# ZooMEISTER/vickers-hardness-Unet

Measured on AMD Instinct MI355X. Metric: 512x512 images/sec (train fwd+bwd), higher is better.
Workload: dtype bf16

## Files before the change

### include/vk_unet.h

```cpp
#ifndef VK_UNET_H
#define VK_UNET_H

#include <stddef.h>
#include <stdint.h>

#ifdef __cplusplus
extern "C" {
#endif

#define VK_ABI_VERSION 1
#define VK_STATS_REPLICAS 32

typedef enum { VK_F32 = 0, VK_BF16 = 1, VK_F16 = 2 } vk_dtype;

enum { VK_OK = 0, VK_ERR_ARG = -1, VK_ERR_STATE = -2, VK_ERR_UNSUPPORTED = -3 };

int vk_version(void);
const char* vk_last_error_string(void);
int vk_has_gfx950_code(void);
int vk_probe_mfma_rate(int iters, int waves_per_simd, float* sink, double* flops_out, void* stream);
int vk_set_reserved_cus(int n);
int vk_debug_hold_cus(int workgroups, int threads, int lds_bytes, int microseconds, const void* traffic, size_t traffic_bytes,
                      float* sink, void* stream);

// ... 377 lines not shown
                               const float* found_inf, float* scratch, void* stream);
#define VK_ADAMW_MAX_GROUPS 8
typedef struct {
  float lr, beta1, beta2, eps, weight_decay;
} vk_adamw_group;
int vk_adamw_step_groups(int n_segments, const int64_t* segments, const int32_t* segment_group, int n_blocks, const int32_t* blocks,
                         float* param, const float* grad, float* exp_avg, float* exp_avg_sq, int n_groups,
                         const vk_adamw_group* groups_host, int* step_counts, float inv_scale, const float* grad_scale,
                         const float* found_inf, const float* clip_coef, float* scratch, void* stream);
#define VK_NORM_L2 0
#define VK_NORM_INF 1
int vk_grad_norm_segments(int n_segments, const int64_t* segments, int n_blocks, const int32_t* blocks, const float* grad,
                          int norm_kind, float inv_scale, float max_norm, double* partials, float* out, void* stream);

typedef struct vk_unet vk_unet;

typedef struct {
  int N, size;
  vk_dtype dtype;
  int training;
  int width;
} vk_unet_config;

typedef struct {
  char name[96];
  int kind;
  int dims[4];
  int ndim;
  int64_t offset;
  int64_t numel;
} vk_tensor_info;

int vk_unet_create(const vk_unet_config* cfg, vk_unet** out);
int vk_unet_create_ex(const vk_unet_config* cfg, int classes, vk_unet** out);
int vk_unet_num_classes(const vk_unet* h);
#define VK_ENC_RESNET18 18
#define VK_ENC_RESNET34 34
#define VK_ENC_RESNET50 50
int vk_unet_create_enc(const vk_unet_config* cfg, int classes, int encoder, vk_unet** out);
int vk_unet_encoder(const vk_unet* h);
void vk_unet_destroy(vk_unet* h);
int vk_unet_set_side_stream(vk_unet* h, int enable);
int vk_unet_num_tensors(const vk_unet* h);
int vk_unet_tensor_info(const vk_unet* h, int index, vk_tensor_info* out);
int64_t vk_unet_param_numel(const vk_unet* h);
int64_t vk_unet_buffer_numel(const vk_unet* h);
int64_t vk_unet_workspace_bytes(const vk_unet* h);
int vk_unet_num_buckets(const vk_unet* h);
int vk_unet_bucket_range(const vk_unet* h, int bucket, int64_t* elem_begin, int64_t* elem_end);

int vk_unet_bind(vk_unet* h, float* params, float* grads, float* bn_buffers, int64_t* nbt, void* workspace,
                 size_t workspace_bytes);
int vk_unet_refresh_weights(vk_unet* h, void* stream);

int vk_unet_forward(vk_unet* h, const float* x, float* logits, int training, void* stream);
int vk_unet_loss(vk_unet* h, const float* logits, const float* target, float* loss_out, float grad_scale,
                 float w_bce, float w_dice, void* stream);
#define VK_LOSS_BINARY 0
#define VK_LOSS_MULTILABEL 1
#define VK_LOSS_MULTICLASS 2
int vk_unet_loss_ex(vk_unet* h, int mode, const void* logits, const void* target, float* loss_out, float grad_scale, float w_ce,
                    float w_dice, void* stream);
int vk_unet_loss_cfg(vk_unet* h, const vk_seg_loss_cfg* cfg, const void* logits, const void* target, float* loss_out,
                     float grad_scale, void* stream);
int vk_unet_loss_lovasz(vk_unet* h, const vk_seg_loss_cfg* seg_cfg, const vk_lovasz_cfg* lovasz_cfg, float w_lovasz, const void* logits,
                        const void* target, void* workspace, size_t workspace_bytes, float* loss_out, float grad_scale, void* stream);
int vk_unet_backward(vk_unet* h, const float* dlogits, int stage_begin, int stage_end, void* stream);
int vk_unet_set_trainable(vk_unet* h, const uint8_t* flags, int n);
int vk_unet_set_bn_frozen(vk_unet* h, const uint8_t* flags, int n);
int vk_unet_set_input_grad(vk_unet* h, float* dx);
int vk_unet_zero_grad(vk_unet* h, void* stream);

#define VK_COMM_ID_BYTES 128
typedef struct vk_comm vk_comm;
int vk_comm_unique_id(void* id_out );
int vk_comm_init(int rank, int world, const void* id, vk_comm** out);
int vk_comm_world(const vk_comm* c);
int vk_allreduce_bucket(vk_comm* c, float* grads, size_t count, void* stream);
int vk_comm_broadcast(vk_comm* c, void* buf, size_t bytes, int root, void* stream);
int vk_comm_destroy(vk_comm* c);

int vk_unet_debug_tensor(const vk_unet* h, const char* name, void** ptr, int dims_nhwc[4]);

#ifdef __cplusplus
}
#endif
#endif
```

### vickers-hardness-unet_amd/_lib.py

```python
from __future__ import annotations

import ctypes as C
import os
import subprocess
from pathlib import Path

PKG_DIR = Path(__file__).resolve().parent
LIB_PATH = Path(os.environ["VK_LIB"]) if os.environ.get("VK_LIB") else PKG_DIR / "libvkunet.so"
CSRC = PKG_DIR / "csrc"

VK_F32, VK_BF16, VK_F16 = 0, 1, 2
VK_LOSS_BINARY, VK_LOSS_MULTILABEL, VK_LOSS_MULTICLASS = 0, 1, 2
VK_ENC_RESNET18, VK_ENC_RESNET34, VK_ENC_RESNET50 = 18, 34, 50
VK_ADAMW_MAX_GROUPS = 8
VK_NORM_L2, VK_NORM_INF = 0, 1
VK_TILE_MAX_ORIGINS, VK_TILE_MAX_SIDE = 64, 4096
VK_BLEND_PROB, VK_BLEND_LOGIT = 0, 1
VK_PATCH_FORCE_GENERAL = 1


class VkError(RuntimeError):
    pass


# ... 4 lines not shown

class vk_conv_desc(C.Structure):
    _fields_ = [("dtype", C.c_int), ("N", C.c_int), ("H", C.c_int), ("W", C.c_int), ("Ho", C.c_int),
                ("Wo", C.c_int), ("K", C.c_int), ("R", C.c_int), ("S", C.c_int), ("stride", C.c_int),
                ("pad", C.c_int), ("transposed", C.c_int), ("src0", vk_src), ("src1", vk_src)]


class vk_bnr(C.Structure):
    _fields_ = [("z", C.c_void_p), ("scale", C.c_void_p), ("shift", C.c_void_p), ("sums", C.c_void_p), ("mask", C.c_void_p),
                ("accumulate", C.c_int)]


class vk_letterbox_desc(C.Structure):
    _fields_ = [("h", C.c_int), ("w", C.c_int), ("src_stride", C.c_int), ("size", C.c_int), ("nh", C.c_int),
                ("nw", C.c_int), ("top", C.c_int), ("left", C.c_int), ("pad_value", C.c_int)]


class vk_tile_desc(C.Structure):
    _fields_ = [("h", C.c_int), ("w", C.c_int), ("src_stride", C.c_int), ("T", C.c_int), ("overlap", C.c_int), ("ny", C.c_int),
                ("nx", C.c_int), ("ys", C.c_int * VK_TILE_MAX_ORIGINS), ("xs", C.c_int * VK_TILE_MAX_ORIGINS), ("view_mask", C.c_int),
                ("pad_value", C.c_int), ("C", C.c_int)]


class vk_geom_desc(C.Structure):
    _fields_ = [("h", C.c_int), ("w", C.c_int), ("bin_thresh", C.c_float), ("morph_kernel", C.c_int), ("open_iter", C.c_int),
                ("close_iter", C.c_int), ("min_area", C.c_int), ("max_components", C.c_int)]


class vk_geom_det(C.Structure):
    _fields_ = [("label", C.c_int), ("area", C.c_int), ("box", C.c_int * 8), ("cx", C.c_float), ("cy", C.c_float),
                ("rw", C.c_float), ("rh", C.c_float), ("ux", C.c_float), ("uy", C.c_float), ("hull_n", C.c_int),
                ("reserved", C.c_int), ("d1", C.c_double), ("d2", C.c_double), ("d_mean", C.c_double)]


class vk_geom_quad(C.Structure):
    _fields_ = [("label", C.c_int), ("area", C.c_int), ("box", C.c_int * 8), ("cx", C.c_float), ("cy", C.c_float),
                ("valid", C.c_int), ("branch", C.c_int), ("n_candidates", C.c_int), ("contour_n", C.c_int), ("hull_n", C.c_int),
                ("flags", C.c_int), ("quality", C.c_double), ("d1", C.c_double), ("d2", C.c_double), ("d_mean", C.c_double)]


class vk_aug_params(C.Structure):
    _fields_ = [("d4", C.c_int), ("rotate", C.c_int), ("cos_a", C.c_float), ("sin_a", C.c_float), ("photo", C.c_int),
                ("alpha", C.c_float), ("beta", C.c_float), ("blur_ksize", C.c_int), ("noise_scale", C.c_float),
                ("noise_seed", C.c_uint32), ("clahe_limit", C.c_int)]


class vk_patch_item(C.Structure):
    _fields_ = [("img_off", C.c_int64), ("msk_off", C.c_int64), ("h", C.c_int), ("w", C.c_int), ("row_off", C.c_int64)]


class vk_patch_params(C.Structure):
    _fields_ = [("item", C.c_int), ("k", C.c_int), ("oy", C.c_int), ("ox", C.c_int), ("zoom", C.c_float), ("cos_a", C.c_float),
                ("sin_a", C.c_float), ("reserved", C.c_int)]


class vk_seg_loss_cfg(C.Structure):
    _fields_ = [("struct_size", C.c_uint32), ("mode", C.c_int32), ("terms", C.c_uint32), ("has_ignore", C.c_int32),
                ("ignore_index", C.c_int32), ("w_pix", C.c_float), ("w_focal", C.c_float), ("w_dice", C.c_float),
                ("w_jaccard", C.c_float), ("w_tversky", C.c_float), ("pix_smooth", C.c_float), ("pix_denom_valid", C.c_int32),
                ("has_pos_weight", C.c_int32), ("pos_weight", C.c_float * 16), ("focal_has_alpha", C.c_int32),
                ("focal_alpha", C.c_float), ("focal_gamma", C.c_float),
                ("dice_smooth", C.c_float), ("dice_eps", C.c_float), ("dice_log", C.c_int32), ("dice_classes", C.c_uint32),
                ("jaccard_smooth", C.c_float), ("jaccard_eps", C.c_float), ("jaccard_log", C.c_int32), ("jaccard_classes", C.c_uint32),
                ("tversky_smooth", C.c_float), ("tversky_eps", C.c_float), ("tversky_log", C.c_int32), ("tversky_classes", C.c_uint32),
                ("tversky_alpha", C.c_float), ("tversky_beta", C.c_float), ("tversky_gamma", C.c_float),
                ("w_mcc", C.c_float), ("mcc_eps", C.c_float)]


class vk_lovasz_cfg(C.Structure):
    _fields_ = [("struct_size", C.c_uint32), ("mode", C.c_int32), ("per_image", C.c_int32), ("has_ignore", C.c_int32),
                ("ignore_index", C.c_int32)]


SWEEP_FIELDS = ("stats", "per_image", "dice", "iou", "mean_dice", "mean_iou", "micro_stats", "micro", "ap", "auc", "best_dice", "best_iou",
                "best_f1", "best_mean", "group_dice", "group_iou", "group_mean_dice", "group_mean_iou", "epoch_dice", "epoch_iou",
                "epoch_mean_dice", "epoch_mean_iou")


class vk_sweep_layout(C.Structure):
    _fields_ = [(f, C.c_size_t) for f in SWEEP_FIELDS + ("total_bytes", "workspace_bytes")]


INST_INT_FIELDS = ("tp", "fp", "fn", "n_rel", "n_pred_used", "n_gt_used", "n_split", "n_merge", "overflow_pred", "overflow_gt", "n_images")
INST_FLOAT_FIELDS = ("sum_iou", "sum_abs_d", "sum_rel_d", "sum_signed_rel_d", "sum_hv_rel", "max_abs_d")


class vk_inst_stats(C.Structure):
    _fields_ = [(f, C.c_int64) for f in INST_INT_FIELDS] + [(f, C.c_double) for f in INST_FLOAT_FIELDS]


VK_SUBPIX_CORNER, VK_SUBPIX_LINES = 0, 1
VK_SUBPIX_MAX_WIN, VK_SUBPIX_MAX_REACH, VK_SUBPIX_MAX_STATIONS = 15, 15, 32
SUBPIX_FLAGS = {"singular": 1, "left_map": 2, "not_converged": 4, "restored": 8, "short_side": 16, "no_edge": 32, "parallel": 64}


class vk_subpix_params(C.Structure):
    _fields_ = [("method", C.c_int), ("win", C.c_int), ("zero_zone", C.c_int), ("max_iter", C.c_int), ("eps", C.c_double),
                ("wt", C.c_double * (2 * VK_SUBPIX_MAX_WIN + 1)), ("n_stations", C.c_int), ("reach", C.c_int), ("lo", C.c_double),
                ("hi", C.c_double), ("level", C.c_double), ("max_shift", C.c_double)]


class vk_subpix_quad(C.Structure):
    _fields_ = [("label", C.c_int), ("area", C.c_int), ("valid", C.c_int), ("reserved", C.c_int), ("flags", C.c_int * 4),
                ("iters", C.c_int * 4), ("v", C.c_double * 8), ("vs", C.c_double * 8), ("d1", C.c_double), ("d2", C.c_double),
                ("d_mean", C.c_double)]

# ... 75 lines not shown
    "vk_head_fwd": (ci, [ci, ci, ci, ci, P(vk_src), vp, vp, vp, vp]),
    "vk_dec4_tail_eval": (ci, [ci, ci, ci, ci, P(vk_src), vp, vp, vp, vp, vp, vp, vp, vp, vp, vp]),
    "vk_head_bwd": (ci, [ci, ci, ci, ci, P(vk_src), vp, vp, vp, vp, vp, vp, sz, vp]),
    "vk_bce_dice_loss": (ci, [sz, vp, vp, vp, vp, vp, cf, cf, cf, vp]),
    "vk_head_fwd_multi": (ci, [ci, ci, ci, ci, ci, P(vk_src), vp, vp, vp, vp]),
    "vk_head_multi_workspace_bytes": (sz, [ci]),
    "vk_head_bwd_multi": (ci, [ci, ci, ci, ci, ci, P(vk_src), vp, vp, vp, vp, vp, P(vk_bnr), vp, sz, vp]),
    "vk_multi_loss_workspace_bytes": (sz, [ci, ci, ci]),
    "vk_multilabel_loss": (ci, [ci, ci, ci, vp, vp, vp, sz, vp, vp, cf, cf, cf, vp]),
    "vk_multiclass_loss": (ci, [ci, ci, ci, vp, vp, vp, sz, vp, vp, cf, cf, cf, vp]),
    "vk_seg_loss_cfg_size": (sz, []),
    "vk_seg_loss_workspace_bytes": (sz, [ci, ci, ci]),
    "vk_seg_loss": (ci, [P(vk_seg_loss_cfg), ci, ci, ci, vp, vp, vp, sz, vp, vp, cf, vp]),
    "vk_lovasz_cfg_size": (sz, []),
    "vk_lovasz_workspace_bytes": (sz, [P(vk_lovasz_cfg), ci, ci, ci]),
    "vk_lovasz_loss": (ci, [P(vk_lovasz_cfg), ci, ci, ci, vp, vp, vp, sz, vp, vp, cf, ci, vp]),
    "vk_lovasz_flat_workspace_bytes": (sz, [ci, i64]),
    "vk_lovasz_flat": (ci, [vp, vp, ci, i64, vp, sz, vp, vp, vp, vp]),
    "vk_seg_metrics_workspace_bytes": (C.c_size_t, [ci]),
    "vk_seg_metrics": (ci, [ci, sz, vp, vp, ci, cf, cf, vp, sz, vp, vp]),
    "vk_seg_metrics_multi_workspace_bytes": (sz, [ci, ci]),
    "vk_seg_metrics_multi": (ci, [ci, ci, ci, sz, vp, vp, ci, cf, cf, vp, sz, vp, vp, vp, vp]),
    "vk_sweep_hist": (ci, [ci, sz, sz, vp, vp, ci, ci, ci, ci, ci, vp, vp, ci, vp, vp, vp]),
    "vk_sweep_curves_layout": (ci, [ci, ci, ci, ci, P(vk_sweep_layout)]),
    "vk_sweep_curves_out_bytes": (sz, [ci, ci, ci, ci]),
    "vk_sweep_curves": (ci, [ci, ci, ci, vp, vp, ci, cf, vp, sz, vp, sz, vp]),
    "vk_inst_contingency": (ci, [ci, ci, ci, vp, vp, ci, ci, vp, vp]),
    "vk_inst_match": (ci, [ci, ci, ci, vp, vp, vp, ci, vp, vp, sz, vp, sz, vp, vp, vp, vp, vp, ci, vp]),
    "vk_subpix_refine": (ci, [P(vk_subpix_params), ci, ci, ci, vp, vp, sz, sz, ci, vp, ci, vp, vp, vp]),
    "vk_adamw_step": (ci, [sz, vp, vp, vp, vp, cf, cf, cf, cf, cf, ci, cf, vp, vp, ci, vp]),
    "vk_amp_check_inf": (ci, [sz, vp, vp, vp]),
    "vk_amp_unscale_check": (ci, [sz, vp, vp, vp, vp]),
    "vk_adamw_step_amp": (ci, [sz, vp, vp, vp, vp, cf, cf, cf, cf, cf, vp, cf, vp, vp, vp, vp, ci, vp]),
    "vk_adamw_segment_blocks": (ci, [ci, P(i64), P(C.c_int32), ci]),
    "vk_adamw_step_amp_segments": (ci, [ci, vp, ci, vp, vp, vp, vp, vp, cf, cf, cf, cf, cf, vp, cf, vp, vp, vp, vp]),
    "vk_adamw_step_groups": (ci, [ci, vp, vp, ci, vp, vp, vp, vp, vp, ci, P(vk_adamw_group), vp, cf, vp, vp, vp, vp, vp]),
    "vk_grad_norm_segments": (ci, [ci, vp, ci, vp, vp, ci, cf, cf, vp, vp, vp]),
    "vk_unet_create": (ci, [P(vk_unet_config), P(vp)]),
    "vk_unet_create_ex": (ci, [P(vk_unet_config), ci, P(vp)]),
    "vk_unet_num_classes": (ci, [vp]),
    "vk_unet_create_enc": (ci, [P(vk_unet_config), ci, ci, P(vp)]),
    "vk_unet_encoder": (ci, [vp]),
    "vk_unet_destroy": (None, [vp]),
    "vk_unet_set_side_stream": (ci, [vp, ci]),
    "vk_unet_num_tensors": (ci, [vp]),
    "vk_unet_tensor_info": (ci, [vp, ci, P(vk_tensor_info)]),
    "vk_unet_param_numel": (i64, [vp]),
    "vk_unet_buffer_numel": (i64, [vp]),
    "vk_unet_workspace_bytes": (i64, [vp]),
    "vk_unet_num_buckets": (ci, [vp]),
    "vk_unet_bucket_range": (ci, [vp, ci, P(i64), P(i64)]),
    "vk_unet_bind": (ci, [vp, vp, vp, vp, vp, vp, sz]),
    "vk_unet_refresh_weights": (ci, [vp, vp]),
    "vk_unet_forward": (ci, [vp, vp, vp, ci, vp]),
    "vk_unet_loss": (ci, [vp, vp, vp, vp, cf, cf, cf, vp]),
    "vk_unet_loss_ex": (ci, [vp, ci, vp, vp, vp, cf, cf, cf, vp]),
    "vk_unet_loss_cfg": (ci, [vp, P(vk_seg_loss_cfg), vp, vp, vp, cf, vp]),
    "vk_unet_loss_lovasz": (ci, [vp, P(vk_seg_loss_cfg), P(vk_lovasz_cfg), cf, vp, vp, vp, sz, vp, cf, vp]),
    "vk_unet_backward": (ci, [vp, vp, ci, ci, vp]),
    "vk_unet_set_trainable": (ci, [vp, P(C.c_uint8), ci]),
    "vk_unet_set_bn_frozen": (ci, [vp, P(C.c_uint8), ci]),
    "vk_unet_set_input_grad": (ci, [vp, vp]),
    "vk_unet_zero_grad": (ci, [vp, vp]),
    "vk_unet_debug_tensor": (ci, [vp, C.c_char_p, P(vp), P(ci * 4)]),
    "vk_comm_unique_id": (ci, [vp]),
    "vk_comm_init": (ci, [ci, ci, vp, P(vp)]),
    "vk_comm_world": (ci, [vp]),
    "vk_allreduce_bucket": (ci, [vp, vp, sz, vp]),
    "vk_comm_broadcast": (ci, [vp, vp, sz, ci, vp]),
    "vk_comm_destroy": (ci, [vp]),
}

_lib = None


def build(force: bool = False, verbose: bool = False) -> Path:
    srcs = list(CSRC.glob("*.hip")) + list(CSRC.glob("*.h")) + [PKG_DIR.parent / "include" / "vk_unet.h"]
    if not force and LIB_PATH.exists() and all(LIB_PATH.stat().st_mtime >= s.stat().st_mtime for s in srcs):
        return LIB_PATH
    hipcc = os.environ.get("HIPCC", "/opt/rocm/bin/hipcc")
    if not Path(hipcc).exists():
        raise VkError(f"hipcc not found at {hipcc}; cannot build libvkunet.so")
    cmd = ["make", "-C", str(CSRC), f"-j{min(4, os.cpu_count() or 1)}", f"HIPCC={hipcc}"]
    r = subprocess.run(cmd, capture_output=True, text=True)
    if verbose:
        print(r.stdout[-2000:], r.stderr[-2000:])
    if r.returncode != 0 or not LIB_PATH.exists():
        raise VkError("building libvkunet.so failed:\n" + r.stdout[-3000:] + r.stderr[-3000:])
    return LIB_PATH


def lib():
    global _lib
    if _lib is not None:
        return _lib
    if not LIB_PATH.exists():
        raise VkError(f"{LIB_PATH} is missing: build it with __graft_entry__.build() "
                      f"(make -C {CSRC}); this package has no CPU fallback")
    try:
        L = C.CDLL(str(LIB_PATH))
    except OSError as e:
        raise VkError(f"cannot load {LIB_PATH}: {e}") from e
    for name, (res, args) in SIGNATURES.items():
        fn = getattr(L, name, None)
        if fn is None:
            raise VkError(f"{LIB_PATH} does not export {name}")
# ... 38 lines not shown
```

### vickers-hardness-unet_amd/csrc/engine.hip

```cpp
#include <stdarg.h>
#include <stdio.h>
#include <stdlib.h>
#include <string.h>

#include <algorithm>
#include <atomic>
#include <map>
#include <mutex>
#include <string>
#include <vector>

#include "vk_common.h"

namespace vkh {
static thread_local char g_err[512] = "";
void set_error(const char* fmt, ...) {
  va_list ap;
  va_start(ap, fmt);
  vsnprintf(g_err, sizeof(g_err), fmt, ap);
  va_end(ap);
}

struct ProfRec {
  std::string tag;
// ... 183 lines not shown
    if (!e.transposed) {
      pos = (int)(v & 3);
      long t = v >> 2;
      k = (int)(t % rows); t /= rows;
      tap = (int)(t % 9); cc = (int)(t / 9);
    } else {
      k = (int)(v % rows);
      long t = v / rows;
      pos = (int)(t & 3); t >>= 2;
      tap = (int)(t % 9); cc = (int)(t / 9);
    }
    const int j = pos ^ (((k >> 2) & 1) << 1);
    const int r0 = cc * CK + j * VE;
    float f[VE];
    if (!e.transposed) {
      const f32x4_t* s4 = reinterpret_cast<const f32x4_t*>(src + ((long)k * 9 + tap) * red + r0);
#pragma unroll
      for (int q = 0; q < VE / 4; ++q) {
        const f32x4_t t = s4[q];
#pragma unroll
        for (int i = 0; i < 4; ++i) f[4 * q + i] = t[i];
      }
    } else {
#pragma unroll
      for (int i = 0; i < VE; ++i) f[i] = src[((long)(r0 + i) * 9 + tap) * rows + k];
    }
    dst[(((long)cc * 9 + tap) * rows + k) * 4 + pos] = Vec16<T>::pack(f);
  }
}

template <typename T>
__global__ void k_cast_flat(size_t n, const float* __restrict__ src, T* __restrict__ dst) {
  for (size_t i = blockIdx.x * (size_t)blockDim.x + threadIdx.x; i < n; i += (size_t)gridDim.x * blockDim.x) st1(dst + i, src[i]);
}

struct CastRange {
  int64_t begin, count;
};
template <typename T>
__global__ void k_cast_ranges(const CastRange* __restrict__ tab, const float* __restrict__ src, T* __restrict__ dst) {
  const CastRange r = tab[blockIdx.y];
  for (int64_t i = blockIdx.x * (int64_t)blockDim.x + threadIdx.x; i < r.count; i += (int64_t)gridDim.x * blockDim.x)
    st1(dst + r.begin + i, src[r.begin + i]);
}

template <typename T>
__global__ void k_pack_stem(const float* __restrict__ w, T* __restrict__ wp) {
  const int i = blockIdx.x * blockDim.x + threadIdx.x;
  if (i >= 64 * 7 * 32) return;
  const int j = i % 32, r = (i / 32) % 7, k = i / (32 * 7);
  const int s = j >> 2, c = j & 3;
  const float v = (s < 7 && c < 3) ? w[((k * 7 + r) * 7 + s) * 3 + c] : 0.f;
  st1(wp + i, v);
}

struct BnEvalEntry {
  int64_t g_off, b_off, rm_off, rv_off, out_off;
  int C, pad_;
};
__global__ void k_bn_eval_all(const BnEvalEntry* __restrict__ tab, const float* __restrict__ params, const float* __restrict__ bufs,
                              float* __restrict__ arena, float eps) {
  const BnEvalEntry e = tab[blockIdx.x];
  for (int c = threadIdx.x; c < e.C; c += blockDim.x) {
    const float invstd = (float)(1.0 / sqrt((double)bufs[e.rv_off + c] + (double)eps));
    const float sc = params[e.g_off + c] * invstd;
    arena[e.out_off + c] = sc;
    arena[e.out_off + e.C + c] = params[e.b_off + c] - bufs[e.rm_off + c] * sc;
  }
}

__global__ void k_inc_i64(int n, int64_t* p) {
  const int i = blockIdx.x * blockDim.x + threadIdx.x;
  if (i < n) p[i] += 1;
}

__global__ void k_inc_i64_masked(int n, int64_t* p, uint64_t frozen) {
  const int i = blockIdx.x * blockDim.x + threadIdx.x;
  if (i < n && !((frozen >> i) & 1ull)) p[i] += 1;
}

__global__ void k_bn_frozen_affine(const BnEvalEntry* __restrict__ tab, uint64_t frozen, const float* __restrict__ params,
                                   const float* __restrict__ bufs, float* __restrict__ arena, float eps) {
  if (!((frozen >> blockIdx.x) & 1ull)) return;
  const BnEvalEntry e = tab[blockIdx.x];
  float* f = arena + e.out_off;
  for (int c = threadIdx.x; c < e.C; c += blockDim.x) {
    const float invstd = (float)(1.0 / sqrt((double)bufs[e.rv_off + c] + (double)eps));
    const float sc = params[e.g_off + c] * invstd;
    f[c] = sc;
    f[e.C + c] = params[e.b_off + c] - bufs[e.rm_off + c] * sc;
    f[2 * e.C + c] = bufs[e.rm_off + c];
    f[3 * e.C + c] = invstd;
    f[4 * e.C + c] = sc;
    f[5 * e.C + c] = 0.f;
    f[6 * e.C + c] = 0.f;
  }
}

struct ConvL {
  std::string name;
  int Cin, K, R, stride, pad;
  int64_t w_off;
  int64_t wd_off;
  bool halo_fwd = false;
  bool halo_dg = false;
  int bn;
// ... 81 lines not shown
  int sink_c = 512;
  int eb;
  std::vector<vk_tensor_info> infos;
  int n_ptensors = 0;
  std::vector<uint8_t> trainable;
  int last_rank = 0;
  uint64_t bn_frozen = 0, bn_frozen_fwd = 0;
  float* dx_in = nullptr;
  int input_rank = 0;
  unsigned mask_version = 0;
  std::vector<ConvL> convs;
  std::vector<BnL> bns;
  std::vector<BlockL> blocks;
  std::vector<DecL> decs;
  int stem_conv = -1, head_conv = -1;
  int layer_last_block[4];
  int64_t n_params = 0, n_bufs = 0, n_dgrad = 0;
  int64_t head_w_off = 0, head_b_off = 0;
  std::vector<std::pair<int64_t, int64_t>> buckets;
  size_t ws_bytes = 0;
  size_t off_x4 = 0, off_pool = 0, off_argmax = 0, off_gpool = 0, off_dup = 0, off_dlogits = 0, off_loss_sums = 0;
  size_t off_stats = 0, off_bsums = 0, stats_bytes = 0, off_farena = 0, farena_floats = 0, off_wf = 0, off_wd = 0, off_wstem = 0;
  size_t off_tab_pack = 0, off_tab_bn = 0, off_wslab = 0, off_wh = 0, off_tab_halo = 0, off_splitk = 0, splitk_bytes = 0;
  std::vector<HaloPackEntry> halo_tab;
  std::vector<size_t> off_z, off_g, off_out, off_gout;
  std::vector<char> g_prereduced;
  std::vector<char> tail_prereduced;
  float* params = nullptr;
  float* grads = nullptr;
  float* bufs = nullptr;
  int64_t* nbt = nullptr;
  char* ws = nullptr;
  bool bound = false;
  hipStream_t side = nullptr;
  hipEvent_t ev_fork = nullptr, ev_join = nullptr;
  bool side_dirty = false;
  struct WItem {
    vk_conv_desc d;
    const void* dz;
    float* dw;
  };
  struct WPlan {
    bool built = false;
    int target = 0, n = 0;
    unsigned version = 0;
    vk::WgradBatchPlan plan;
  };
  std::vector<WItem> pending;
  WPlan wplans[kMaxStages][2];
  size_t off_tab_wbatch = 0;
  std::vector<PackEntry> pack_tab;
  std::vector<CastRange> cast_tab;
  size_t off_tab_cast = 0;
  size_t off_gscratch = 0;
  size_t off_sloss = 0, sloss_bytes = 0;
  size_t off_mloss = 0, mloss_bytes = 0;
  std::vector<BnEvalEntry> bn_tab;
  std::map<std::string, std::pair<void*, std::vector<int>>> debug;

  int N() const { return cfg.N; }
};

namespace {

size_t align_up(size_t v, size_t a) { return (v + a - 1) / a * a; }

bool need_from(const vk_unet* h, int rank) { return h->last_rank >= rank; }
bool trains(const vk_unet* h, int t) { return h->trainable[(size_t)t] != 0; }
bool frozen(const vk_unet* h, const BnL& b) { return (h->bn_frozen_fwd >> b.idx) & 1ull; }
bool bn_sums_needed(const vk_unet* h, const BnL& b) { return !frozen(h, b) || trains(h, b.g_t) || trains(h, b.b_t); }
float* grad_or_sink(vk_unet* h, int t, int64_t off, int sink_off) {
  return trains(h, t) ? h->grads + off : (float*)(h->ws + h->off_gscratch) + sink_off;
}
float* dgamma_of(vk_unet* h, const BnL& b) { return grad_or_sink(h, b.g_t, b.g_off, 0); }
float* dbeta_of(vk_unet* h, const BnL& b) { return grad_or_sink(h, b.b_t, b.b_off, h->sink_c); }

int add_info(vk_unet* h, const std::string& name, int kind, std::vector<int> dims, int64_t offset, int64_t numel) {
  vk_tensor_info ti;
  memset(&ti, 0, sizeof(ti));
  snprintf(ti.name, sizeof(ti.name), "%s", name.c_str());
  ti.kind = kind;
  ti.ndim = (int)dims.size();
  for (size_t i = 0; i < dims.size() && i < 4; ++i) ti.dims[i] = dims[i];
  ti.offset = offset;
  ti.numel = numel;
  h->infos.push_back(ti);
  return kind <= 1 ? h->n_ptensors++ : -1;
}

int add_conv(vk_unet* h, const std::string& name, int Cin, int K, int R, int stride, int pad, int Hin, int Win, bool bias = false) {
  ConvL c;
  c.name = name;
  c.Cin = Cin; c.K = K; c.R = R; c.stride = stride; c.pad = pad;
  c.Hin = Hin; c.Win = Win;
  c.Hout = (Hin + 2 * pad - R) / stride + 1;
  c.Wout = (Win + 2 * pad - R) / stride + 1;
  c.w_off = h->n_params;
  c.wd_off = -1;
  c.bn = -1;
  const int64_t numel = (int64_t)K * Cin * R * R;
  c.w_t = add_info(h, name + ".weight", 0, {K, Cin, R, R}, c.w_off, numel);
  h->n_params += (int64_t)align_up((size_t)numel, 4);
  if (bias) {
    c.b_t = add_info(h, name + ".bias", 1, {K}, h->n_params, K);
    h->n_params += (int64_t)align_up((size_t)K, 4);
  }
// ... 113 lines not shown
    const int64_t end = hi + 1 < (int)block_start.size() ? block_start[(size_t)hi + 1] : dec_start[0];
    h->buckets.push_back({s + 1 == E.nstages ? 0 : block_start[(size_t)lo], end});
  }
}

void assign_backward_ranks(vk_unet* h) {
  int r = 0;
  auto conv = [&](int i) { h->convs[(size_t)i].rank = r++; };
  auto bn = [&](int i) { h->bns[(size_t)h->convs[(size_t)i].bn].rank = r++; };
  conv(h->head_conv);
  for (int i = 4; i >= 0; --i) {
    const DecL& d = h->decs[(size_t)i];
    bn(d.conv2); conv(d.conv2); bn(d.conv1); conv(d.conv1);
  }
  for (int bi = (int)h->blocks.size() - 1; bi >= 0; --bi) {
    const BlockL& k = h->blocks[(size_t)bi];
    if (k.conv3 >= 0) {
      bn(k.conv3);
      if (k.convd >= 0) bn(k.convd);
      conv(k.conv3);
      if (k.convd >= 0) conv(k.convd);
      bn(k.conv2); conv(k.conv2);
      bn(k.conv1); conv(k.conv1);
      continue;
    }
    bn(k.conv2);
    if (k.convd >= 0) bn(k.convd);
    conv(k.conv2);
    if (k.convd >= 0) conv(k.convd);
    bn(k.conv1); conv(k.conv1);
  }
  bn(h->stem_conv); conv(h->stem_conv);
  h->input_rank = r;
  h->trainable.assign((size_t)h->n_ptensors, 1);
  h->last_rank = r - 1;
}

void update_last_rank(vk_unet* h) {
  h->last_rank = -1;
  for (const ConvL& c : h->convs) {
    if (trains(h, c.w_t) || (c.b_t >= 0 && trains(h, c.b_t))) h->last_rank = std::max(h->last_rank, c.rank);
  }
  for (const BnL& b : h->bns) {
    if (trains(h, b.g_t) || trains(h, b.b_t)) h->last_rank = std::max(h->last_rank, b.rank);
  }
  if (h->dx_in) h->last_rank = h->input_rank;
}

size_t grad_scratch_floats(const vk_unet* h) {
  if (h->enc->code != VK_ENC_RESNET34) return align_up(2 * (size_t)h->sink_c + 145 * (size_t)h->classes, 64);
  return h->classes == 1 ? kGradScratchFloats : align_up(1024 + 145 * (size_t)h->classes, 64);
}

void layout_workspace(vk_unet* h) {
  const int N = h->cfg.N, S = h->cfg.size, SW = h->cfg.width, eb = h->eb;
  const bool tr = h->cfg.training != 0;
  size_t off = 0;
  auto take = [&](size_t bytes) {
    const size_t o = off;
    off = align_up(off + bytes, 256);
    return o;
  };
  h->off_x4 = take((size_t)N * S * SW * 4 * eb);
  h->g_prereduced.assign(h->convs.size(), 0);
  h->tail_prereduced.assign(h->blocks.size(), 0);
  h->off_z.resize(h->convs.size());
  h->off_g.assign(h->convs.size(), 0);
  for (size_t i = 0; i < h->convs.size(); ++i) {
    const ConvL& c = h->convs[i];
    if ((int)i == h->head_conv) { h->off_z[i] = 0; continue; }
    const size_t bytes = (size_t)N * c.Hout * c.Wout * c.K * eb;
    h->off_z[i] = take(bytes);
    if (tr) h->off_g[i] = take(bytes);
  }
  h->off_pool = take((size_t)N * (S / 4) * (SW / 4) * 64 * eb);
  h->off_argmax = take((size_t)N * (S / 4) * (SW / 4) * 64);
  if (tr) h->off_gpool = take((size_t)N * (S / 4) * (SW / 4) * 64 * eb);
  h->off_out.resize(h->blocks.size());
  h->off_gout.assign(h->blocks.size(), 0);
  for (size_t b = 0; b < h->blocks.size(); ++b) {
    const BlockL& k = h->blocks[b];
    const size_t bytes = (size_t)N * k.Hout * k.Wout * k.C * eb;
    h->off_out[b] = take(bytes);
    if (tr) h->off_gout[b] = take(bytes);
  }
  if (tr) {
    size_t mx = 0;
    for (const DecL& d : h->decs) mx = std::max(mx, (size_t)N * d.H * d.W * d.Cup * eb);
    h->off_dup = take(mx);
    h->off_dlogits = take((size_t)N * h->classes * S * SW * 4);
  }
  h->off_loss_sums = take(8 * sizeof(double));
  size_t st = 0, fl = 0;
  for (BnL& b : h->bns) {
    st += 2 * (size_t)b.C * sizeof(double) * VK_STATS_REPLICAS;
    b.arena_off = (int64_t)fl;
    fl += 7 * (size_t)b.C;
  }
  h->stats_bytes = st;
  h->off_stats = take(st);
  h->off_bsums = take(st);
  h->farena_floats = fl;
  h->off_farena = take(fl * sizeof(float));
  h->off_wf = (eb == 4) ? 0 : take((size_t)h->n_params * eb);
  h->off_wd = tr ? take((size_t)h->n_dgrad * eb) : 0;
  h->off_wh = take((size_t)h->n_params * eb);
  h->off_tab_halo = take(2 * h->convs.size() * sizeof(HaloPackEntry));
  h->off_wstem = take(64 * 7 * 32 * eb);
  h->off_wslab = tr ? take(kEngineSlabBytes) : 0;
  h->off_tab_wbatch = tr ? take((size_t)kMaxStages * 2 * VK_WGRAD_BATCH_TABLE_BYTES) : 0;
  h->splitk_bytes = (!tr && (size_t)N * S * SW <= 4u * 512 * 512) ? VK_SPLITK_WORKSPACE_BYTES : 0;
  h->off_splitk = h->splitk_bytes ? take(h->splitk_bytes) : 0;
  h->off_tab_pack = take(h->convs.size() * sizeof(PackEntry));
  h->off_tab_cast = take(h->convs.size() * sizeof(CastRange));
  h->off_tab_bn = take(h->bns.size() * sizeof(BnEvalEntry));
  h->off_gscratch = tr ? take(grad_scratch_floats(h) * sizeof(float)) : 0;
  if (h->classes > 1) {
    h->mloss_bytes = vk_multi_loss_workspace_bytes(N, h->classes, S * SW);
    h->off_mloss = take(h->mloss_bytes);
  }
  h->sloss_bytes = vk_seg_loss_workspace_bytes(N, h->classes, S * SW);
  h->off_sloss = take(h->sloss_bytes);
  h->ws_bytes = off;
}

void assign_pointers(vk_unet* h) {
  char* ws = h->ws;
  h->debug.clear();
  const int N = h->cfg.N;
  for (size_t i = 0; i < h->convs.size(); ++i) {
    ConvL& c = h->convs[i];
    if ((int)i == h->head_conv) continue;
    c.z = ws + h->off_z[i];
    c.g = h->cfg.training ? ws + h->off_g[i] : nullptr;
    h->debug["z:" + c.name] = {c.z, {N, c.Hout, c.Wout, c.K}};
    if (c.g) h->debug["g:" + c.name] = {c.g, {N, c.Hout, c.Wout, c.K}};
  }
  for (size_t b = 0; b < h->blocks.size(); ++b) {
    BlockL& k = h->blocks[b];
    k.out = ws + h->off_out[b];
    k.gout = h->cfg.training ? ws + h->off_gout[b] : nullptr;
    const std::string nm = h->convs[k.conv1].name.substr(0, h->convs[k.conv1].name.size() - 6);
    h->debug["out:" + nm] = {k.out, {N, k.Hout, k.Wout, k.C}};
    if (k.gout) h->debug["gout:" + nm] = {k.gout, {N, k.Hout, k.Wout, k.C}};
  }
  const int S = h->cfg.size, SW = h->cfg.width;
  h->debug["x4"] = {ws + h->off_x4, {N, S, SW, 4}};
  h->debug["pool"] = {ws + h->off_pool, {N, S / 4, SW / 4, 64}};
  if (h->cfg.training) {
    h->debug["gpool"] = {ws + h->off_gpool, {N, S / 4, SW / 4, 64}};
    if (h->classes == 1) h->debug["dlogits"] = {ws + h->off_dlogits, {N, S, SW, 1}};
    else h->debug["dlogits"] = {ws + h->off_dlogits, {N, h->classes, S, SW}};
  }
  double* sp = (double*)(ws + h->off_stats);
  double* bp = (double*)(ws + h->off_bsums);
  float* fa = (float*)(ws + h->off_farena);
  for (BnL& b : h->bns) {
    b.stats = sp;
    b.bsums = bp;
    sp += 2 * b.C * VK_STATS_REPLICAS;
    bp += 2 * b.C * VK_STATS_REPLICAS;
    float* f = fa + b.arena_off;
    b.scale = f;
    b.shift = f + b.C;
    b.mean = f + 2 * b.C;
    b.invstd = f + 3 * b.C;
    b.coef = f + 4 * b.C;
    h->debug["scale:" + b.name] = {b.scale, {b.C}};
    h->debug["shift:" + b.name] = {b.shift, {b.C}};
  }
}

const void* fwd_weights(const vk_unet* h, const ConvL& c) {
  if (c.halo_fwd) return h->ws + h->off_wh + (size_t)c.w_off * h->eb;
  if (h->eb == 4) return h->params + c.w_off;
// ... 98 lines not shown
  VK_CHECK_ARG(cfg->N >= 1 && cfg->size >= 32 && cfg->size % 32 == 0 && width >= 32 && width % 32 == 0,
               "Wrong input shape height=%d, width=%d: must be divisible by 32", cfg->size, width);
  VK_CHECK_ARG(cfg->dtype == VK_F32 || cfg->dtype == VK_BF16 || cfg->dtype == VK_F16, "vk_unet_create: bad dtype");
  vk_unet* h = new vk_unet();
  h->cfg = *cfg;
  h->classes = classes;
  h->enc = enc;
  h->cfg.width = width;
  h->eb = cfg->dtype == VK_F32 ? 4 : 2;
  build_topology(h);
  if (enc->code != VK_ENC_RESNET34)
    for (const BnL& b : h->bns) h->sink_c = std::max(h->sink_c, b.C);
  if ((int)h->bns.size() > kMaxBnLayers) {
    delete h;
    vkh::set_error("vk_unet_create_enc: more BatchNorm layers than the frozen-statistics mask holds");
    return VK_ERR_ARG;
  }
  assign_backward_ranks(h);
  layout_workspace(h);
  *out = h;
  return VK_OK;
}

extern "C" int vk_unet_num_classes(const vk_unet* h) { return h ? h->classes : 0; }
extern "C" int vk_unet_encoder(const vk_unet* h) { return h ? h->enc->code : 0; }

extern "C" void vk_unet_destroy(vk_unet* h) {
  if (!h) return;
  if (h->side) {
    (void)hipStreamSynchronize(h->side);
    (void)hipEventDestroy(h->ev_fork);
    (void)hipEventDestroy(h->ev_join);
    (void)hipStreamDestroy(h->side);
  }
  delete h;
}
extern "C" int vk_unet_num_tensors(const vk_unet* h) { return h ? (int)h->infos.size() : 0; }
extern "C" int vk_unet_tensor_info(const vk_unet* h, int index, vk_tensor_info* out) {
  VK_CHECK_ARG(h && out && index >= 0 && index < (int)h->infos.size(), "vk_unet_tensor_info: bad index %d", index);
  *out = h->infos[index];
  return VK_OK;
}
extern "C" int64_t vk_unet_param_numel(const vk_unet* h) { return h ? h->n_params : 0; }
extern "C" int64_t vk_unet_buffer_numel(const vk_unet* h) { return h ? h->n_bufs : 0; }
extern "C" int64_t vk_unet_workspace_bytes(const vk_unet* h) { return h ? (int64_t)h->ws_bytes : 0; }
extern "C" int vk_unet_num_buckets(const vk_unet* h) { return h ? (int)h->buckets.size() : 0; }
extern "C" int vk_unet_bucket_range(const vk_unet* h, int bucket, int64_t* b, int64_t* e) {
  VK_CHECK_ARG(h && b && e && bucket >= 0 && bucket < (int)h->buckets.size(), "vk_unet_bucket_range: bad bucket %d", bucket);
  *b = h->buckets[bucket].first;
  *e = h->buckets[bucket].second;
  return VK_OK;
}

extern "C" int vk_unet_bind(vk_unet* h, float* params, float* grads, float* bn_buffers, int64_t* nbt, void* workspace,
                            size_t workspace_bytes) {
  VK_CHECK_ARG(h && params && bn_buffers && nbt && workspace, "vk_unet_bind: null argument");
  VK_CHECK_ARG(!h->cfg.training || grads, "vk_unet_bind: a training plan needs a gradient buffer");
  VK_CHECK_ARG(workspace_bytes >= h->ws_bytes, "vk_unet_bind: workspace too small (%zu < %zu)", workspace_bytes, h->ws_bytes);
  VK_CHECK_ARG(((uintptr_t)workspace & 255) == 0 && ((uintptr_t)params & 15) == 0, "vk_unet_bind: buffers must be 256-byte (workspace) / 16-byte (params) aligned");
  h->params = params; h->grads = grads; h->bufs = bn_buffers; h->nbt = nbt; h->ws = (char*)workspace;
  for (auto& st_ : h->wplans) { st_[0].built = false; st_[1].built = false; }
  h->pending.clear();
  assign_pointers(h);
  h->halo_tab.clear();
  {
    auto plain = [&](int C) { vk_src s = null_src(); s.ptr = h->ws; s.C = C; return s; };
    auto fwd_uses = [&](ConvL& c, int C0, int C1, int up) {
      vk_src s0 = plain(C0), s1 = C1 ? plain(C1) : null_src();
      s0.up = up;
      vk_conv_desc d = conv_desc(h, c, s0, s1);
      return vk_conv_uses_halo_pack(&d) != 0;
    };
    for (size_t i = 0; i < h->convs.size(); ++i) {
      ConvL& c = h->convs[i];
      c.halo_fwd = c.halo_dg = false;
      if ((int)i == h->stem_conv || (int)i == h->head_conv) continue;
      c.halo_fwd = fwd_uses(c, c.Cin, 0, 0);
    }
    for (DecL& d : h->decs) {
      ConvL& c = h->convs[d.conv1];
      c.halo_fwd = fwd_uses(c, d.Cup, d.Cskip, 1);
    }
    for (size_t i = 0; i < h->convs.size(); ++i) {
      ConvL& c = h->convs[i];
      if (c.wd_off >= 0 && h->cfg.training) {
        vk_conv_desc d;
        d.dtype = h->cfg.dtype;
        d.N = h->cfg.N; d.H = c.Hout; d.W = c.Wout; d.Ho = c.Hin; d.Wo = c.Win;
        d.K = c.Cin; d.R = c.R; d.S = c.R; d.stride = c.stride; d.pad = c.pad; d.transposed = 1;
        d.src0 = plain(c.K);
        d.src1 = null_src();
        c.halo_dg = vk_conv_uses_halo_pack(&d) != 0;
      }
      HaloPackEntry e;
      e.src = c.w_off; e.pad_ = 0;
      if (c.halo_fwd) {
        e.dst = (int64_t)(h->off_wh + (size_t)c.w_off * h->eb); e.rows = c.K; e.red = c.Cin; e.transposed = 0;
        h->halo_tab.push_back(e);
      }
      if (c.halo_dg) {
        e.dst = (int64_t)(h->off_wd + (size_t)c.wd_off * h->eb); e.rows = c.Cin; e.red = c.K; e.transposed = 1;
        h->halo_tab.push_back(e);
      }
    }
  }
  h->pack_tab.clear();
  for (size_t i = 0; i < h->convs.size(); ++i) {
    const ConvL& c = h->convs[i];
    if (c.wd_off < 0 || c.halo_dg) continue;
    PackEntry e;
    e.src = c.w_off; e.dst = c.wd_off; e.K = c.K; e.RS = c.R * c.R; e.C = c.Cin; e.pad_ = 0;
    h->pack_tab.push_back(e);
  }
  h->cast_tab.clear();
  for (size_t i = 0; i < h->convs.size(); ++i) {
    const ConvL& c = h->convs[i];
    if ((int)i == h->stem_conv || (int)i == h->head_conv || c.halo_fwd) continue;
    h->cast_tab.push_back(CastRange{c.w_off, (int64_t)c.K * c.Cin * c.R * c.R});
  }
  h->bn_tab.clear();
  for (const BnL& b : h->bns) {
    BnEvalEntry e;
    e.g_off = b.g_off; e.b_off = b.b_off; e.rm_off = b.rm_off; e.rv_off = b.rv_off; e.out_off = b.arena_off; e.C = b.C; e.pad_ = 0;
    h->bn_tab.push_back(e);
  }
  if (!h->pack_tab.empty())
    VK_CHECK_HIP(hipMemcpy(h->ws + h->off_tab_pack, h->pack_tab.data(), h->pack_tab.size() * sizeof(PackEntry), hipMemcpyHostToDevice));
  if (!h->halo_tab.empty())
    VK_CHECK_HIP(hipMemcpy(h->ws + h->off_tab_halo, h->halo_tab.data(), h->halo_tab.size() * sizeof(HaloPackEntry), hipMemcpyHostToDevice));
  if (!h->cast_tab.empty())
    VK_CHECK_HIP(hipMemcpy(h->ws + h->off_tab_cast, h->cast_tab.data(), h->cast_tab.size() * sizeof(CastRange), hipMemcpyHostToDevice));
  VK_CHECK_HIP(hipMemcpy(h->ws + h->off_tab_bn, h->bn_tab.data(), h->bn_tab.size() * sizeof(BnEvalEntry), hipMemcpyHostToDevice));
  if (h->cfg.training && !h->side && getenv("VK_SIDE_STREAM")) RET_IF(vk_unet_set_side_stream(h, 1));
  h->bound = true;
  return VK_OK;
}

template <typename T>
static int refresh_t(vk_unet* h, hipStream_t st) {
  vkh::ProfScope ps_("weights_repack", st, 0.0, (double)h->n_params * (4.0 + 2.0 * sizeof(T)));
  if (sizeof(T) != 4 && !h->cast_tab.empty())
    hipLaunchKernelGGL(k_cast_ranges<T>, dim3(16, (unsigned)h->cast_tab.size()), dim3(256), 0, st, (const CastRange*)(h->ws + h->off_tab_cast),
                       h->params, (T*)(h->ws + h->off_wf));
  if (h->cfg.training && !h->pack_tab.empty())
    hipLaunchKernelGGL(k_pack_dgrad<T>, dim3(64, (unsigned)h->pack_tab.size()), dim3(256), 0, st,
                       (const PackEntry*)(h->ws + h->off_tab_pack), h->params, (T*)(h->ws + h->off_wd));
  if (!h->halo_tab.empty())
    hipLaunchKernelGGL(k_pack_halo_tab<T>, dim3(32, (unsigned)h->halo_tab.size()), dim3(256), 0, st,
                       (const HaloPackEntry*)(h->ws + h->off_tab_halo), h->params, h->ws);
  hipLaunchKernelGGL(k_pack_stem<T>, dim3((64 * 7 * 32 + 255) / 256), dim3(256), 0, st,
                     h->params + h->convs[h->stem_conv].w_off, (T*)(h->ws + h->off_wstem));
  VK_CHECK_HIP(hipGetLastError());
  return VK_OK;
}

extern "C" int vk_unet_refresh_weights(vk_unet* h, void* stream) {
  VK_CHECK_ARG(h && h->bound, "vk_unet_refresh_weights: plan not bound");
  hipStream_t st = (hipStream_t)stream;
  switch (h->cfg.dtype) {
    case VK_F32: return refresh_t<float>(h, st);
    case VK_BF16: return refresh_t<bf16_t>(h, st);
    case VK_F16: return refresh_t<f16_t>(h, st);
  }
  return VK_ERR_ARG;
}

extern "C" int vk_unet_set_side_stream(vk_unet* h, int enable) {
  VK_CHECK_ARG(h, "vk_unet_set_side_stream: null plan");
  if (enable && !h->side && h->cfg.training) {
    VK_CHECK_HIP(hipStreamCreateWithFlags(&h->side, hipStreamNonBlocking));
    VK_CHECK_HIP(hipEventCreateWithFlags(&h->ev_fork, hipEventDisableTiming));
    VK_CHECK_HIP(hipEventCreateWithFlags(&h->ev_join, hipEventDisableTiming));
  } else if (!enable && h->side) {
    VK_CHECK_HIP(hipStreamSynchronize(h->side));
    (void)hipEventDestroy(h->ev_fork);
    (void)hipEventDestroy(h->ev_join);
    (void)hipStreamDestroy(h->side);
    h->side = nullptr;
    h->ev_fork = h->ev_join = nullptr;
    h->side_dirty = false;
  }
  return VK_OK;
}

extern "C" int vk_unet_set_trainable(vk_unet* h, const uint8_t* flags, int n) {
  VK_CHECK_ARG(h && flags, "vk_unet_set_trainable: null argument");
  VK_CHECK_ARG(n == h->n_ptensors, "vk_unet_set_trainable: %d flags for %d parameter tensors", n, h->n_ptensors);
  bool changed = false;
  for (int t = 0; t < n; ++t) {
    const uint8_t v = flags[t] ? 1 : 0;
    changed |= v != h->trainable[(size_t)t];
    h->trainable[(size_t)t] = v;
  }
// ... 633 lines not shown
```

Measured before the change: 3082.

## Fuse weight cast, dgrad, halo and stem packing into one unit-table kernel

Replaces the four separate weight repack launches (range cast, dgrad transpose, halo pack, stem pack) with a single kernel driven by a host-built table of 32x32 tile units. Each unit reads an fp32 weight tile once, stages it in LDS, and writes every required layout (cast, transposed dgrad, swizzled halo forward/dgrad). The aim is to cut launch count and repeated reads of the fp32 parameters during each per-step weight refresh. The cost is a more complex kernel with added layout constraints checked at bind, plus a new table-export API. The old path stays available behind an environment variable.

```diff
diff --git a/include/vk_unet.h b/include/vk_unet.h
--- a/include/vk_unet.h
+++ b/include/vk_unet.h
@@ -453,6 +453,12 @@
 int vk_unet_bind(vk_unet* h, float* params, float* grads, float* bn_buffers, int64_t* nbt, void* workspace,
                  size_t workspace_bytes);
 int vk_unet_refresh_weights(vk_unet* h, void* stream);
+typedef struct vk_pack_layer {
+  int64_t src;
+  int64_t dst_fwd, dst_dg, dst_cast, dst_t;
+  int K, RS, C, kind;
+} vk_pack_layer;
+int vk_unet_pack_table(vk_unet* h, vk_pack_layer* layers, int layer_capacity, int32_t* units, int unit_capacity, int* n_units);
 
 int vk_unet_forward(vk_unet* h, const float* x, float* logits, int training, void* stream);
 int vk_unet_loss(vk_unet* h, const float* logits, const float* target, float* loss_out, float grad_scale,
diff --git a/vickers-hardness-unet_amd/_lib.py b/vickers-hardness-unet_amd/_lib.py
--- a/vickers-hardness-unet_amd/_lib.py
+++ b/vickers-hardness-unet_amd/_lib.py
@@ -80,6 +80,11 @@
 class vk_patch_params(C.Structure):
     _fields_ = [("item", C.c_int), ("k", C.c_int), ("oy", C.c_int), ("ox", C.c_int), ("zoom", C.c_float), ("cos_a", C.c_float),
                 ("sin_a", C.c_float), ("reserved", C.c_int)]
+
+
+class vk_pack_layer(C.Structure):
+    _fields_ = [("src", C.c_int64), ("dst_fwd", C.c_int64), ("dst_dg", C.c_int64), ("dst_cast", C.c_int64), ("dst_t", C.c_int64),
+                ("K", C.c_int), ("RS", C.c_int), ("C", C.c_int), ("kind", C.c_int)]
 
 
 class vk_seg_loss_cfg(C.Structure):
@@ -261,6 +266,7 @@
     "vk_unet_bucket_range": (ci, [vp, ci, P(i64), P(i64)]),
     "vk_unet_bind": (ci, [vp, vp, vp, vp, vp, vp, sz]),
     "vk_unet_refresh_weights": (ci, [vp, vp]),
+    "vk_unet_pack_table": (ci, [vp, P(vk_pack_layer), ci, P(C.c_int32), ci, P(ci)]),
     "vk_unet_forward": (ci, [vp, vp, vp, ci, vp]),
     "vk_unet_loss": (ci, [vp, vp, vp, vp, cf, cf, cf, vp]),
     "vk_unet_loss_ex": (ci, [vp, ci, vp, vp, vp, cf, cf, cf, vp]),
diff --git a/vickers-hardness-unet_amd/csrc/engine.hip b/vickers-hardness-unet_amd/csrc/engine.hip
--- a/vickers-hardness-unet_amd/csrc/engine.hip
+++ b/vickers-hardness-unet_amd/csrc/engine.hip
@@ -259,6 +259,107 @@
   const int s = j >> 2, c = j & 3;
   const float v = (s < 7 && c < 3) ? w[((k * 7 + r) * 7 + s) * 3 + c] : 0.f;
   st1(wp + i, v);
+}
+
+struct PackLayer {
+  int64_t src;
+  int64_t dst_fwd;
+  int64_t dst_dg;
+  int64_t dst_cast;
+  int64_t dst_t;
+  int K, RS, C, kind;
+};
+static_assert(sizeof(PackLayer) == sizeof(vk_pack_layer), "PackLayer mirrors vk_pack_layer");
+constexpr int kPackUnitsPerWg = 2;
+constexpr int kStemPackElems = 64 * 7 * 32;
+
+template <typename T>
+__global__ __launch_bounds__(256) void k_pack_units(const PackLayer* __restrict__ layers, const int2* __restrict__ units, int n_units,
+                                                    const float* __restrict__ params, char* __restrict__ ws) {
+  constexpr int VE = ElemTraits<T>::kVec, CK = 64 / ElemTraits<T>::kBytes, NV = 1024 / VE, U = kPackUnitsPerWg;
+  __shared__ float tl[U][32][33];
+  const int tid = threadIdx.x;
+  PackLayer e[U];
+  int k0[U], c0[U], tap[U];
+  bool on[U];
+  f32x4_t v[U];
+#pragma unroll
+  for (int i = 0; i < U; ++i) {
+    const int idx = blockIdx.x * U + i;
+    on[i] = idx < n_units;
+    const int2 u = units[on[i] ? idx : n_units - 1];
+    e[i] = layers[u.x];
+    if (e[i].kind == 1) {
+      const int o = u.y * 256 + tid;
+      if (on[i] && o < kStemPackElems) {
+        const int j = o % 32, r = (o / 32) % 7, k = o / (32 * 7);
+        const int s = j >> 2, c = j & 3;
+        const float f = (s < 7 && c < 3) ? params[e[i].src + ((k * 7 + r) * 7 + s) * 3 + c] : 0.f;
+        st1(reinterpret_cast<T*>(ws + e[i].dst_fwd) + o, f);
+      }
+      on[i] = false;
+      continue;
+    }
+    const int ct_n = (e[i].C + 31) / 32;
+    c0[i] = (u.y % ct_n) * 32;
+    const int rem = u.y / ct_n;
+    tap[i] = rem % e[i].RS;
+    k0[i] = (rem / e[i].RS) * 32;
+    const int k = k0[i] + (tid >> 3), c = c0[i] + (tid & 7) * 4;
+    v[i] = f32x4_t{0.f, 0.f, 0.f, 0.f};
+    if (on[i] && k < e[i].K && c < e[i].C)
+      v[i] = *reinterpret_cast<const f32x4_t*>(params + e[i].src + (unsigned)((k * e[i].RS + tap[i]) * e[i].C + c));
+  }
+#pragma unroll
+  for (int i = 0; i < U; ++i) {
+    if (!on[i]) continue;
+    const int r = tid >> 3, cl = (tid & 7) * 4;
+#pragma unroll
+    for (int q = 0; q < 4; ++q) tl[i][r][cl + q] = v[i][q];
+    const int k = k0[i] + r, c = c0[i] + cl;
+    if (e[i].dst_cast >= 0 && k < e[i].K && c < e[i].C) {
+      T* d = reinterpret_cast<T*>(ws + e[i].dst_cast) + (unsigned)((k * e[i].RS + tap[i]) * e[i].C + c);
+#pragma unroll
+      for (int q = 0; q < 4; ++q) st1(d + q, v[i][q]);
+    }
+  }
+  __syncthreads();
+#pragma unroll
+  for (int i = 0; i < U; ++i) {
+    if (!on[i]) continue;
+    const int K = e[i].K, C = e[i].C, t = tap[i];
+    if (e[i].dst_t >= 0) {
+      T* d = reinterpret_cast<T*>(ws + e[i].dst_t);
+      const int tx = tid & 31, ty = tid >> 5;
+#pragma unroll
+      for (int q = 0; q < 4; ++q) {
+        const int c = c0[i] + ty + 8 * q, k = k0[i] + tx;
+        if (k < K && c < C) st1(d + (unsigned)((c * e[i].RS + t) * K + k), tl[i][tx][ty + 8 * q]);
+      }
+    }
+    if (tid < NV) {
+      const int pos = tid & 3, rl = (tid >> 2) & 31, hl = (tid >> 7) * CK;
+      float f[VE];
+      if (e[i].dst_fwd >= 0) {
+        const int k = k0[i] + rl, cb = c0[i] + hl;
+        if (k < K && cb < C) {
+          const int j = pos ^ (((k >> 2) & 1) << 1);
+#pragma unroll
+          for (int q = 0; q < VE; ++q) f[q] = tl[i][rl][hl + j * VE + q];
+          reinterpret_cast<u32x4_t*>(ws + e[i].dst_fwd)[(unsigned)((((cb / CK) * 9 + t) * K + k) * 4 + pos)] = Vec16<T>::pack(f);
+        }
+      }
+      if (e[i].dst_dg >= 0) {
+        const int c = c0[i] + rl, kb = k0[i] + hl;
+        if (c < C && kb < K) {
+          const int j = pos ^ (((c >> 2) & 1) << 1);
+#pragma unroll
+          for (int q = 0; q < VE; ++q) f[q] = tl[i][hl + j * VE + q][rl];
+          reinterpret_cast<u32x4_t*>(ws + e[i].dst_dg)[(unsigned)((((kb / CK) * 9 + t) * C + c) * 4 + pos)] = Vec16<T>::pack(f);
+        }
+      }
+    }
+  }
 }
 
 struct BnEvalEntry {
@@ -446,6 +547,9 @@
   std::vector<PackEntry> pack_tab;
   std::vector<CastRange> cast_tab;
   size_t off_tab_cast = 0;
+  std::vector<PackLayer> pk_layers;
+  std::vector<int32_t> pk_units;
+  size_t off_tab_pk_layers = 0, off_tab_pk_units = 0, pk_units_cap = 0;
   size_t off_gscratch = 0;
   size_t off_sloss = 0, sloss_bytes = 0;
   size_t off_mloss = 0, mloss_bytes = 0;
@@ -665,6 +769,12 @@
   return h->classes == 1 ? kGradScratchFloats : align_up(1024 + 145 * (size_t)h->classes, 64);
 }
 
+size_t pack_unit_count(const vk_unet* h, int i) {
+  const ConvL& c = h->convs[(size_t)i];
+  if (i == h->stem_conv) return (kStemPackElems + 255) / 256;
+  return (size_t)((c.K + 31) / 32) * ((c.Cin + 31) / 32) * c.R * c.R;
+}
+
 void layout_workspace(vk_unet* h) {
   const int N = h->cfg.N, S = h->cfg.size, SW = h->cfg.width, eb = h->eb;
   const bool tr = h->cfg.training != 0;
@@ -734,6 +844,11 @@
   }
   h->sloss_bytes = vk_seg_loss_workspace_bytes(N, h->classes, S * SW);
   h->off_sloss = take(h->sloss_bytes);
+  h->pk_units_cap = 0;
+  for (size_t i = 0; i < h->convs.size(); ++i)
+    if ((int)i != h->head_conv) h->pk_units_cap += pack_unit_count(h, (int)i);
+  h->off_tab_pk_layers = take(h->convs.size() * sizeof(PackLayer));
+  h->off_tab_pk_units = take(h->pk_units_cap * 2 * sizeof(int32_t));
   h->ws_bytes = off;
 }
 
@@ -938,19 +1053,11 @@
   return VK_OK;
 }
 
-extern "C" int vk_unet_bind(vk_unet* h, float* params, float* grads, float* bn_buffers, int64_t* nbt, void* workspace,
-                            size_t workspace_bytes) {
-  VK_CHECK_ARG(h && params && bn_buffers && nbt && workspace, "vk_unet_bind: null argument");
-  VK_CHECK_ARG(!h->cfg.training || grads, "vk_unet_bind: a training plan needs a gradient buffer");
-  VK_CHECK_ARG(workspace_bytes >= h->ws_bytes, "vk_unet_bind: workspace too small (%zu < %zu)", workspace_bytes, h->ws_bytes);
-  VK_CHECK_ARG(((uintptr_t)workspace & 255) == 0 && ((uintptr_t)params & 15) == 0, "vk_unet_bind: buffers must be 256-byte (workspace) / 16-byte (params) aligned");
-  h->params = params; h->grads = grads; h->bufs = bn_buffers; h->nbt = nbt; h->ws = (char*)workspace;
-  for (auto& st_ : h->wplans) { st_[0].built = false; st_[1].built = false; }
-  h->pending.clear();
-  assign_pointers(h);
+static int build_weight_tables(vk_unet* h) {
   h->halo_tab.clear();
   {
-    auto plain = [&](int C) { vk_src s = null_src(); s.ptr = h->ws; s.C = C; return s; };
+    static char some_tensor;
+    auto plain = [&](int C) { vk_src s = null_src(); s.ptr = &some_tensor; s.C = C; return s; };
     auto fwd_uses = [&](ConvL& c, int C0, int C1, int up) {
       vk_src s0 = plain(C0), s1 = C1 ? plain(C1) : null_src();
       s0.up = up;
@@ -1004,6 +1111,67 @@
     if ((int)i == h->stem_conv || (int)i == h->head_conv || c.halo_fwd) continue;
     h->cast_tab.push_back(CastRange{c.w_off, (int64_t)c.K * c.Cin * c.R * c.R});
   }
+  h->pk_layers.clear();
+  h->pk_units.clear();
+  const size_t eb = (size_t)h->eb;
+  for (size_t i = 0; i < h->convs.size(); ++i) {
+    const ConvL& c = h->convs[i];
+    if ((int)i == h->head_conv) continue;
+    PackLayer e;
+    e.src = c.w_off; e.dst_fwd = e.dst_dg = e.dst_cast = e.dst_t = -1;
+    e.K = c.K; e.RS = c.R * c.R; e.C = c.Cin; e.kind = 0;
+    if ((int)i == h->stem_conv) {
+      e.kind = 1;
+      e.dst_fwd = (int64_t)h->off_wstem;
+    } else {
+      if (c.halo_fwd) e.dst_fwd = (int64_t)(h->off_wh + (size_t)c.w_off * eb);
+      else if (eb != 4) e.dst_cast = (int64_t)(h->off_wf + (size_t)c.w_off * eb);
+      if (c.halo_dg) e.dst_dg = (int64_t)(h->off_wd + (size_t)c.wd_off * eb);
+      else if (c.wd_off >= 0 && h->cfg.training) e.dst_t = (int64_t)(h->off_wd + (size_t)c.wd_off * eb);
+      if (e.dst_fwd < 0 && e.dst_dg < 0 && e.dst_cast < 0 && e.dst_t < 0) continue;
+      const int ck = 64 / (int)eb;
+      VK_CHECK_ARG((int64_t)c.K * e.RS * c.Cin < (1 << 28), "weight pack: layer %s is too large for 32-bit offsets", c.name.c_str());
+      VK_CHECK_ARG(c.Cin % 4 == 0 && (e.dst_fwd < 0 || (e.RS == 9 && c.Cin % ck == 0)) && (e.dst_dg < 0 || (e.RS == 9 && c.K % ck == 0)),
+                   "weight pack: layer %s (%d x %d x %d) does not fit the unit kernel", c.name.c_str(), c.K, e.RS, c.Cin);
+    }
+    const size_t n = pack_unit_count(h, (int)i);
+    for (size_t t = 0; t < n; ++t) {
+      h->pk_units.push_back((int32_t)h->pk_layers.size());
+      h->pk_units.push_back((int32_t)t);
+    }
+    h->pk_layers.push_back(e);
+  }
+  VK_CHECK_ARG(h->pk_units.size() / 2 <= h->pk_units_cap, "weight pack: %zu units exceed the %zu laid out", h->pk_units.size() / 2, h->pk_units_cap);
+  return VK_OK;
+}
+
+extern "C" int vk_unet_pack_table(vk_unet* h, vk_pack_layer* layers, int layer_capacity, int32_t* units, int unit_capacity, int* n_units) {
+  VK_CHECK_ARG(h && n_units && layer_capacity >= 0 && unit_capacity >= 0, "vk_unet_pack_table: bad argument");
+  if (!h->bound) RET_IF(build_weight_tables(h));
+  const int nl = (int)h->pk_layers.size(), nu = (int)(h->pk_units.size() / 2);
+  *n_units = nu;
+  if (layers) {
+    VK_CHECK_ARG(nl <= layer_capacity, "vk_unet_pack_table: %d layers do not fit in %d", nl, layer_capacity);
+    memcpy(layers, h->pk_layers.data(), (size_t)nl * sizeof(PackLayer));
+  }
+  if (units) {
+    VK_CHECK_ARG(nu <= unit_capacity, "vk_unet_pack_table: %d units do not fit in %d", nu, unit_capacity);
+    memcpy(units, h->pk_units.data(), (size_t)nu * 2 * sizeof(int32_t));
+  }
+  return nl;
+}
+
+extern "C" int vk_unet_bind(vk_unet* h, float* params, float* grads, float* bn_buffers, int64_t* nbt, void* workspace,
+                            size_t workspace_bytes) {
+  VK_CHECK_ARG(h && params && bn_buffers && nbt && workspace, "vk_unet_bind: null argument");
+  VK_CHECK_ARG(!h->cfg.training || grads, "vk_unet_bind: a training plan needs a gradient buffer");
+  VK_CHECK_ARG(workspace_bytes >= h->ws_bytes, "vk_unet_bind: workspace too small (%zu < %zu)", workspace_bytes, h->ws_bytes);
+  VK_CHECK_ARG(((uintptr_t)workspace & 255) == 0 && ((uintptr_t)params & 15) == 0, "vk_unet_bind: buffers must be 256-byte (workspace) / 16-byte (params) aligned");
+  h->params = params; h->grads = grads; h->bufs = bn_buffers; h->nbt = nbt; h->ws = (char*)workspace;
+  for (auto& st_ : h->wplans) { st_[0].built = false; st_[1].built = false; }
+  h->pending.clear();
+  assign_pointers(h);
+  RET_IF(build_weight_tables(h));
   h->bn_tab.clear();
   for (const BnL& b : h->bns) {
     BnEvalEntry e;
@@ -1016,6 +1184,10 @@
     VK_CHECK_HIP(hipMemcpy(h->ws + h->off_tab_halo, h->halo_tab.data(), h->halo_tab.size() * sizeof(HaloPackEntry), hipMemcpyHostToDevice));
   if (!h->cast_tab.empty())
     VK_CHECK_HIP(hipMemcpy(h->ws + h->off_tab_cast, h->cast_tab.data(), h->cast_tab.size() * sizeof(CastRange), hipMemcpyHostToDevice));
+  if (!h->pk_units.empty()) {
+    VK_CHECK_HIP(hipMemcpy(h->ws + h->off_tab_pk_layers, h->pk_layers.data(), h->pk_layers.size() * sizeof(PackLayer), hipMemcpyHostToDevice));
+    VK_CHECK_HIP(hipMemcpy(h->ws + h->off_tab_pk_units, h->pk_units.data(), h->pk_units.size() * sizeof(int32_t), hipMemcpyHostToDevice));
+  }
   VK_CHECK_HIP(hipMemcpy(h->ws + h->off_tab_bn, h->bn_tab.data(), h->bn_tab.size() * sizeof(BnEvalEntry), hipMemcpyHostToDevice));
   if (h->cfg.training && !h->side && getenv("VK_SIDE_STREAM")) RET_IF(vk_unet_set_side_stream(h, 1));
   h->bound = true;
@@ -1025,6 +1197,15 @@
 template <typename T>
 static int refresh_t(vk_unet* h, hipStream_t st) {
   vkh::ProfScope ps_("weights_repack", st, 0.0, (double)h->n_params * (4.0 + 2.0 * sizeof(T)));
+  if (!getenv("VK_PACK_SPLIT")) {
+    const int n_units = (int)(h->pk_units.size() / 2);
+    if (n_units)
+      hipLaunchKernelGGL(k_pack_units<T>, dim3((unsigned)((n_units + kPackUnitsPerWg - 1) / kPackUnitsPerWg)), dim3(256), 0, st,
+                         (const PackLayer*)(h->ws + h->off_tab_pk_layers), (const int2*)(h->ws + h->off_tab_pk_units), n_units, h->params,
+                         h->ws);
+    VK_CHECK_HIP(hipGetLastError());
+    return VK_OK;
+  }
   if (sizeof(T) != 4 && !h->cast_tab.empty())
     hipLaunchKernelGGL(k_cast_ranges<T>, dim3(16, (unsigned)h->cast_tab.size()), dim3(256), 0, st, (const CastRange*)(h->ws + h->off_tab_cast),
                        h->params, (T*)(h->ws + h->off_wf));
```

New measurement: 3108, median of 6. Within noise of the previous version (+0.8%).
